# Ensembl/WiggleTools

Hardware: AMD Instinct MI355X
Metric: genomic bp/s (whole node) for 'mean' over N BigWig tracks (higher is better)
Workload: dtype f64

## Files before the change

include/wiggletools_amd.h:

```cpp
#ifndef WIGGLETOOLS_AMD_H_
#define WIGGLETOOLS_AMD_H_

#include <stdint.h>
#include <stdio.h>

#ifdef __cplusplus
extern "C" {
#endif


typedef char wt_bool;

typedef struct wiggleIterator_st WiggleIterator;
typedef struct multiplexer_st Multiplexer;
typedef struct multiset_st Multiset;

struct wiggleIterator_st {
    char *chrom;
    int start;
    int finish;
    double value;
    void *valuePtr;
    wt_bool done;
    int strand;
// ... 147 lines not shown
void wtamd_warmup_async(void);
const char *wtamd_last_error(void);
const char *wtamd_version(void);

#define WTAMD_MAX_COORD (2147483647 - 65536)

int wtamd_trackset_create_host(const wtamd_tracks *tracks, wtamd_trackset **out);
int wtamd_trackset_create_device(const wtamd_tracks *tracks, wtamd_trackset **out);
void wtamd_trackset_destroy(wtamd_trackset *);

int wtamd_trackset_validate(wtamd_trackset *ts, int64_t *n_bad, int64_t *first_bad);

int64_t wtamd_trackset_max_runs(const wtamd_trackset *ts);

int wtamd_trackset_index(wtamd_trackset *ts, int op, void *stream);

int wtamd_reduce(wtamd_trackset *ts, const wtamd_reduce_desc *desc, wtamd_runs *runs,
                 int64_t *n_runs, void *stream);

int wtamd_reduce_host(wtamd_trackset *ts, const wtamd_reduce_desc *desc, wtamd_runs *runs,
                      int64_t *n_runs);

int wtamd_multiplex_host(wtamd_trackset *ts, uint32_t flags, wtamd_runs *runs,
                         double *values, uint8_t *inplay, int64_t *n_runs);

int wtamd_runs_auc(const wtamd_runs *runs, int64_t n_runs, double *auc, void *stream);
int wtamd_runs_mean(const wtamd_runs *runs, int64_t n_runs, double *mean, void *stream);

int wtamd_pearson(wtamd_trackset *ts, double *result);
int wtamd_pearson_moments(wtamd_trackset *ts, double *moments6);
// ... 304 lines not shown
```

wiggletools_amd/_lib.py:

```python
import ctypes as C
import os

_HERE = os.path.dirname(os.path.abspath(__file__))
LIB_PATH = os.environ.get("WTAMD_LIB") or os.path.join(_HERE, "csrc", "libwiggletools_amd.so")


class Tracks(C.Structure):
    _fields_ = [("n_chrom", C.c_int32), ("n_tracks", C.c_int32), ("seg_off", C.c_void_p),
                ("start", C.c_void_p), ("finish", C.c_void_p), ("value", C.c_void_p),
                ("value_is_f64", C.c_int32), ("defaults", C.c_void_p),
                ("range_lo", C.c_void_p), ("range_hi", C.c_void_p)]


class ReduceDesc(C.Structure):
    _fields_ = [("op", C.c_int32), ("flags", C.c_uint32), ("n_set0", C.c_int32), ("reserved", C.c_int32)]


class Runs(C.Structure):
    _fields_ = [("capacity", C.c_int64), ("start", C.c_void_p), ("finish", C.c_void_p),
                ("value", C.c_void_p), ("chrom_run_off", C.c_void_p)]


class Stats(C.Structure):
    _fields_ = [("n_runs", C.c_int64), ("covered_bp", C.c_int64), ("n_intervals", C.c_int64),
# ... 15 lines not shown
    try:
        if os.environ.get("WTAMD_NO_TORCH"):
            raise ImportError
        import torch
    except ImportError:
        pass
    L = C.CDLL(LIB_PATH)
    L.wtamd_last_error.restype = C.c_char_p
    L.wtamd_version.restype = C.c_char_p
    L.wtamd_device_count.restype = C.c_int
    L.wtamd_set_device.argtypes = [C.c_int]
    L.wtamd_trackset_create_host.argtypes = [C.POINTER(Tracks), C.POINTER(C.c_void_p)]
    L.wtamd_trackset_create_device.argtypes = [C.POINTER(Tracks), C.POINTER(C.c_void_p)]
    L.wtamd_trackset_destroy.argtypes = [C.c_void_p]
    L.wtamd_trackset_destroy.restype = None
    L.wtamd_trackset_max_runs.argtypes = [C.c_void_p]
    L.wtamd_trackset_max_runs.restype = C.c_int64
    L.wtamd_trackset_index.argtypes = [C.c_void_p, C.c_int, C.c_void_p]
    L.wtamd_reduce.argtypes = [C.c_void_p, C.POINTER(ReduceDesc), C.POINTER(Runs), C.POINTER(C.c_int64), C.c_void_p]
    L.wtamd_reduce_host.argtypes = [C.c_void_p, C.POINTER(ReduceDesc), C.POINTER(Runs), C.POINTER(C.c_int64)]
    L.wtamd_multiplex_host.argtypes = [C.c_void_p, C.c_uint32, C.POINTER(Runs), C.c_void_p, C.c_void_p,
                                       C.POINTER(C.c_int64)]
    L.wtamd_runs_auc.argtypes = [C.POINTER(Runs), C.c_int64, C.POINTER(C.c_double), C.c_void_p]
    L.wtamd_runs_map.argtypes = [C.c_int, C.c_double, C.c_int64, C.c_void_p, C.c_void_p, C.c_void_p, C.c_void_p, C.c_int,
                                 C.c_void_p, C.c_void_p, C.c_void_p, C.c_void_p, C.c_void_p]
    L.wtamd_runs_coverage.argtypes = [C.c_int64, C.c_void_p, C.c_void_p, C.c_void_p, C.c_int64, C.c_void_p, C.c_void_p, C.c_void_p,
                                      C.c_void_p, C.POINTER(C.c_int64), C.c_void_p]
    L.wtamd_runs_union.argtypes = [C.c_int64, C.c_void_p, C.c_void_p, C.c_void_p, C.c_void_p, C.c_int, C.c_int64, C.c_void_p, C.c_void_p,
                                   C.c_void_p, C.c_void_p, C.POINTER(C.c_int64), C.c_void_p]
    L.wtamd_runs_region.argtypes = [C.c_int, C.c_int64, C.c_void_p, C.c_void_p, C.c_void_p, C.c_void_p, C.c_int, C.c_void_p, C.c_void_p,
# ... 70 lines not shown
```

wiggletools_amd/csrc/wt_engine.hip:

```cpp
#include <hip/hip_runtime.h>

#include <cstdio>
#include <thread>
#include <atomic>
#include <cstring>
#include <map>
#include <mutex>
#include <string>
#include <vector>

#include "wt_host.h"
#include "wt_trackset.h"
#include "wt_core.h"
#include "wt_plan.h"
#include "wt_kernels.h"
#include "wt_devscope.h"
#include "wt_pool.h"

#ifndef WT_INDEX_UNROLL
#define WT_INDEX_UNROLL 2
#endif
#define WT_INDEX_CHUNK (256 * 4 * WT_INDEX_UNROLL)
__global__ void __launch_bounds__(256) wt_index_kernel(const WtParams P, long long total, long long span) {
    const long long dev_total = P.seg_off[(long long) P.n_chrom * P.n_tracks];
    if (total > dev_total) total = dev_total;
    const long long begin0 = (long long) blockIdx.x * span;
    long long end0 = begin0 + span;
    if (end0 > total) end0 = total;
    if (begin0 >= end0) return;
    WtIndexCursor cur;
    wt_index_cursor_set(P, cur, wt_index_find_segment(P, begin0));
    struct __attribute__((packed, aligned(4))) V4 { int32_t x[4]; };
    V4 f[WT_INDEX_UNROLL], nf[WT_INDEX_UNROLL];
    int32_t pf[WT_INDEX_UNROLL], npf[WT_INDEX_UNROLL];
    const long long n_full = (end0 - begin0) / WT_INDEX_CHUNK;
    auto fetch = [&](long long base, V4 (&v)[WT_INDEX_UNROLL], int32_t (&p)[WT_INDEX_UNROLL]) {
#pragma unroll
        for (int u = 0; u < WT_INDEX_UNROLL; u++) {
// ... 29 lines not shown
            const long long g = begin + 4ll * (threadIdx.x + 256 * u);
            int32_t prev = (g < end0 && g > 0) ? P.finish[g - 1] : 0;
#pragma unroll
            for (int q = 0; q < 4; q++) {
                if (g + q < end0) {
                    const int32_t fq = P.finish[g + q];
                    wt_index_apply(P, cur, g + q, fq, prev);
                    prev = fq;
                }
            }
        }
    }
}

#define WT_ISEARCH_ROWS 64
#define WT_ISEARCH_TRACKS 16

__device__ __forceinline__ int wt_index_row_chrom(const WtParams &P, long long row) {
    int lo = 0;
    for (int hi = P.n_chrom; hi - lo > 1;) {
        const int mid = (lo + hi) >> 1;
        if (P.c_first_win[mid] + mid <= row) lo = mid; else hi = mid;
    }
    return lo;
}

struct WtIndexRow { int ch; long long b, s0, n; };
__device__ __forceinline__ WtIndexRow wt_index_row(const WtParams &P, long long row, int i) {
    WtIndexRow r;
    r.ch = P.n_chrom == 1 ? 0 : wt_index_row_chrom(P, row);
    const long long m = row - (P.c_first_win[r.ch] + r.ch);
    const long long seg = (long long) r.ch * P.n_tracks + i;
    r.s0 = P.seg_off[seg];
    r.n = P.seg_off[seg + 1] - r.s0;
    r.b = (long long) P.cbase[r.ch] + (m << P.logW);
    return r;
}

__global__ void __launch_bounds__(256) wt_index_coarse_kernel(const WtParams P, long long n_strips, uint32_t *coarse) {
    const long long t = (long long) blockIdx.x * 256 + threadIdx.x;
    const int N = P.n_tracks;
    if (t >= n_strips * N) return;
    const long long strip = t / N;
    const int i = (int) (t - strip * N);
    const WtIndexRow r = wt_index_row(P, strip * WT_ISEARCH_ROWS, i);
    const int32_t *fin = P.finish + r.s0;
    long long g = r.n >> 1;
    float density = 0.0f;
    if (r.n > 1) {
        const long long f0 = fin[0], f1 = fin[r.n - 1];
        if (f1 > f0) {
            density = (float) (r.n - 1) / (float) (f1 - f0);
            const float guess = fminf(fmaxf((float) (r.b - f0) * density, 0.0f), (float) (r.n - 1));
            g = (long long) guess;
            if (g > r.n - 1) g = r.n - 1;
        }
    }
    coarse[t] = (uint32_t) wt_interp_lower_bound(WtFinArray{fin}, 0, r.n, g, r.b, density);
}

__global__ void __launch_bounds__(WT_ISEARCH_ROWS * WT_ISEARCH_TRACKS) wt_index_search_kernel(const WtParams P, long long n_rows, long long n_strips,
                                                                                              const uint32_t *coarse) {
    __shared__ uint32_t out[WT_ISEARCH_ROWS][WT_ISEARCH_TRACKS + 1];
    const int tid = threadIdx.x, lane = tid & 63;
    const int wave = __builtin_amdgcn_readfirstlane(tid >> 6);
    const int N = P.n_tracks;
    const long long strip = blockIdx.x;
    const long long r0 = strip * WT_ISEARCH_ROWS;
    const int i = (int) blockIdx.y * WT_ISEARCH_TRACKS + wave;
    if (i < N) {
        long long row = r0 + lane;
        if (row > n_rows - 1) row = n_rows - 1;
        const WtIndexRow r = wt_index_row(P, row, i);
        const int32_t *fin = P.finish + r.s0;
        const bool have_next = strip + 1 < n_strips;
        const long long cA = (long long) coarse[strip * N + i];
        const long long cB = have_next ? (long long) coarse[(strip + 1) * N + i] : 0;
        bool real_a = true, real_b = have_next;
// ... 14 lines not shown
    const long long row = r0 + orow;
    const int track = (int) blockIdx.y * WT_ISEARCH_TRACKS + ocol;
    if (row < n_rows && track < N) P.widx[(size_t) row * N + track] = out[orow][ocol];
}

__global__ void __launch_bounds__(256) wt_index_compare_kernel(const uint32_t *a, const uint32_t *b, long long n, unsigned long long *diff) {
    const long long t = (long long) blockIdx.x * 256 + threadIdx.x;
    if (t < n && a[t] != b[t]) atomicAdd(diff, 1ull);
}

__global__ void __launch_bounds__(256) wt_extents_kernel(const int64_t *seg_off, const int32_t *start,
                                                          const int32_t *finish, long long n_seg,
                                                          int32_t *first_start, int32_t *last_finish) {
    const long long s = (long long) blockIdx.x * blockDim.x + threadIdx.x;
    if (s >= n_seg) return;
    const long long lo = seg_off[s], hi = seg_off[s + 1];
    first_start[s] = hi > lo ? start[lo] : 0;
    last_finish[s] = hi > lo ? finish[hi - 1] : 0;
}

__global__ void __launch_bounds__(256) wt_win_chrom_kernel(const int64_t *c_first_win, int n_chrom, long long n_windows, int32_t *win_chrom) {
    const long long k = (long long) blockIdx.x * 256 + threadIdx.x;
    if (k >= n_windows) return;
    int lo = 0;
    for (int hi = n_chrom; hi - lo > 1;) {
        const int mid = (lo + hi) >> 1;
        if (c_first_win[mid] <= k) lo = mid; else hi = mid;
    }
    win_chrom[k] = lo;
}

__global__ void __launch_bounds__(256) wt_clear_kernel(unsigned long long *counters, int n_counters, int64_t *chrom_run_off, int n_cro,
                                                        unsigned long long *status, long long n_status) {
    const long long t = (long long) blockIdx.x * 256 + threadIdx.x, stride = (long long) gridDim.x * 256;
    for (long long q = t; q < n_status; q += stride) status[q] = 0ull;
    for (long long q = t; q < n_counters; q += stride) counters[q] = 0ull;
    for (long long q = t; q < n_cro; q += stride) chrom_run_off[q] = 0;
}

__global__ void __launch_bounds__(256) wt_validate_kernel(const int32_t *start, const int32_t *finish, const int64_t *seg_off,
                                                           long long n_seg, long long total, unsigned long long *out) {
    const long long g = (long long) blockIdx.x * blockDim.x + threadIdx.x;
    if (g >= total) return;
    bool bad = finish[g] <= start[g];
    if (!bad && g > 0 && start[g] < finish[g - 1]) {
        long long lo = 0, hi = n_seg;
        while (hi - lo > 1) {
            const long long mid = (lo + hi) >> 1;
            if (seg_off[mid] <= g) lo = mid; else hi = mid;
        }
        bad = seg_off[lo] != g;
// ... 137 lines not shown
    WT_HIP(hipEventCreate(&ts->ev_r0));
    WT_HIP(hipEventCreate(&ts->ev_r1));
    return WTAMD_OK;
}

extern "C++" int wt_check_extents(wtamd_trackset *ts) {
    for (size_t q = 0; q < ts->last_finish.size(); q++)
        if (ts->seg_off[q + 1] > ts->seg_off[q] && ts->last_finish[q] > WTAMD_MAX_COORD) {
            const int64_t bad = ts->last_finish[q];
            return wt_fail(WTAMD_ERR_ARG, "run finish " + std::to_string(bad) + " above the supported maximum " +
                           std::to_string((long long) WTAMD_MAX_COORD) + " (2^31 - 65537)");
        }
    return WTAMD_OK;
}

static int wt_refresh_extents_device(wtamd_trackset *ts, hipStream_t s) {
    const int64_t n_seg = (int64_t) ts->n_chrom * ts->n_tracks;
    ts->first_start.assign(n_seg, 0);
    ts->last_finish.assign(n_seg, 0);
    if (n_seg > 0 && ts->n_intervals > 0) {
        const size_t bytes = sizeof(int32_t) * 2 * (size_t) n_seg;
        if (!ts->d_extents) WT_HIP(wt_dev_alloc(&ts->d_extents, bytes));
        if (!ts->h_extents) WT_HIP(wt_host_alloc((void **) &ts->h_extents, bytes));
        hipLaunchKernelGGL(wt_extents_kernel, dim3((unsigned) ((n_seg + 255) / 256)), dim3(256), 0, s,
                           ts->d_seg_off, ts->d_start, ts->d_finish, (long long) n_seg, ts->d_extents, ts->d_extents + n_seg);
        WT_HIP(hipGetLastError());
        WT_HIP(hipMemcpyAsync(ts->h_extents, ts->d_extents, bytes, hipMemcpyDeviceToHost, s));
        WT_HIP(hipStreamSynchronize(s));
        ts->first_start.assign(ts->h_extents, ts->h_extents + n_seg);
        ts->last_finish.assign(ts->h_extents + n_seg, ts->h_extents + 2 * n_seg);
    }
    return WTAMD_OK;
}

static int wt_create_host_impl(const wtamd_tracks *t, wtamd_trackset *ts) {
    int rc = wt_trackset_common(t, ts);
    if (rc != WTAMD_OK) return rc;
    ts->owns = true;
// ... 26 lines not shown
    const int rc = wt_create_host_impl(t, ts);
    if (rc != WTAMD_OK) { wtamd_trackset_destroy(ts); return rc; }
    *out = ts;
    return WTAMD_OK;
}

static int wt_create_device_impl(const wtamd_tracks *t, wtamd_trackset *ts) {
    int rc = wt_trackset_common(t, ts);
    if (rc != WTAMD_OK) return rc;
    ts->owns = false;
    ts->d_start = const_cast<int32_t *>(t->start);
    ts->d_finish = const_cast<int32_t *>(t->finish);
    ts->d_value = const_cast<void *>(t->value);
    rc = wt_refresh_extents_device(ts, nullptr);
    if (rc != WTAMD_OK) return rc;
    return wt_check_extents(ts);
}

int wtamd_trackset_create_device(const wtamd_tracks *t, wtamd_trackset **out) {
    if (!out) return wt_fail(WTAMD_ERR_ARG, "out == NULL");
    wtamd_trackset *ts = new wtamd_trackset();
    const int rc = wt_create_device_impl(t, ts);
    if (rc != WTAMD_OK) { wtamd_trackset_destroy(ts); return rc; }
    *out = ts;
    return WTAMD_OK;
}

void wtamd_trackset_destroy(wtamd_trackset *ts) {
    if (!ts) return;
    (void) wt_pool_quiesce();
    if (ts->owns) { (void) hipFree(ts->d_start); (void) hipFree(ts->d_finish); (void) hipFree(ts->d_value); }
    (void) wt_dev_free(ts->d_seg_off); (void) wt_dev_free(ts->d_defaults); (void) wt_dev_free(ts->d_counters); (void) wt_dev_free(ts->d_chrom_run_off);
    (void) wt_dev_free(ts->d_extents);
    (void) hipFree(ts->d_gscratch); (void) hipFree(ts->d_mwu_table);
    for (double *q : ts->mwu_retired) (void) hipFree(q);
    if (ts->h_counters) wt_host_free(ts->h_counters);
    if (ts->h_debug) wt_host_free(ts->h_debug);
    if (ts->h_extents) wt_host_free(ts->h_extents);
    for (auto &kv : ts->windows) wt_free_windows(kv.second);
    if (ts->ev_i0) (void) hipEventDestroy(ts->ev_i0);
    if (ts->ev_i1) (void) hipEventDestroy(ts->ev_i1);
    if (ts->ev_r0) (void) hipEventDestroy(ts->ev_r0);
    if (ts->ev_r1) (void) hipEventDestroy(ts->ev_r1);
    delete ts;
}

static int64_t wt_span(const wtamd_trackset *ts) {
    int64_t span = 0;
    for (int c = 0; c < ts->n_chrom; c++) {
        int64_t lo = INT64_MAX, hi = INT64_MIN;
        for (int i = 0; i < ts->n_tracks; i++) {
            const int64_t s = (int64_t) c * ts->n_tracks + i;
            if (ts->seg_off[s + 1] > ts->seg_off[s]) {
                lo = std::min<int64_t>(lo, ts->first_start[s]);
                hi = std::max<int64_t>(hi, ts->last_finish[s]);
            }
        }
        if (lo <= hi) span += hi - lo;
    }
    return span;
}

int64_t wtamd_trackset_max_runs(const wtamd_trackset *ts) {
    if (!ts) return 0;
    return std::min<int64_t>(2 * ts->n_intervals, wt_span(ts));
}

static int wt_get_windows(wtamd_trackset *ts, int W, WtWindows **out, hipStream_t s = nullptr) {
    WtWindows &w = ts->windows[W];
    *out = &w;
    if (w.tab_valid) return WTAMD_OK;
    wt_make_windows(ts->n_chrom, ts->n_tracks, ts->seg_off.data(), ts->first_start.data(), ts->last_finish.data(), W, w.tab,
                    ts->range_lo.empty() ? nullptr : ts->range_lo.data(),
                    ts->range_hi.empty() ? nullptr : ts->range_hi.data(), false);
    w.indexed = false;
    const int64_t nc = ts->n_chrom > 0 ? ts->n_chrom : 1;
    const int64_t nwin = w.tab.n_windows > 0 ? w.tab.n_windows : 1;
    const int64_t nwidx = (w.tab.n_rows > 0 ? w.tab.n_rows : 1) * (int64_t) ts->n_tracks;
    auto up8 = [](int64_t x) { return (x + 7) & ~(int64_t) 7; };
// ... 28 lines not shown
            w.h_tab = nullptr; w.h_tab_bytes = 0;
            WT_HIP(wt_host_alloc((void **) &w.h_tab, (size_t) head));
            w.h_tab_bytes = head;
        }
        const int64_t o_cfirst = (char *) w.d_cfirst - w.d_tabs;
        const int64_t used = o_cfirst + (int64_t) sizeof(int64_t) * (ts->n_chrom + 1);
        memset(w.h_tab, 0, (size_t) used);
        memcpy(w.h_tab + ((char *) w.d_cbase - w.d_tabs), w.tab.cbase.data(), sizeof(int32_t) * ts->n_chrom);
        memcpy(w.h_tab + ((char *) w.d_cnwin - w.d_tabs), w.tab.c_nwin.data(), sizeof(int32_t) * ts->n_chrom);
        memcpy(w.h_tab + ((char *) w.d_chi - w.d_tabs), w.tab.c_hi.data(), sizeof(int32_t) * ts->n_chrom);
        memcpy(w.h_tab + o_cfirst, w.tab.c_first_win.data(), sizeof(int64_t) * (ts->n_chrom + 1));
        WT_HIP(hipMemcpyAsync(w.d_tabs, w.h_tab, (size_t) used, hipMemcpyHostToDevice, s));
        WT_HIP(hipEventRecord(w.ev_tab, s));
        w.tab_in_flight = true;
        if (w.tab.n_windows > 0) {
            if (ts->n_chrom == 1) {
                WT_HIP(hipMemsetAsync(w.d_win_chrom, 0, sizeof(int32_t) * (size_t) w.tab.n_windows, s));
            } else {
                hipLaunchKernelGGL(wt_win_chrom_kernel, dim3((unsigned) ((w.tab.n_windows + 255) / 256)), dim3(256), 0, s,
                                   (const int64_t *) w.d_cfirst, ts->n_chrom, (long long) w.tab.n_windows, w.d_win_chrom);
                WT_HIP(hipGetLastError());
            }
        }
    }
    w.tab_valid = true;
    return WTAMD_OK;
}

static void wt_fill_params(const wtamd_trackset *ts, const WtWindows *w, const WtPlan &plan, WtParams &P) {
    memset(&P, 0, sizeof(P));
    P.start = ts->d_start; P.finish = ts->d_finish; P.value = ts->d_value;
    P.seg_off = ts->d_seg_off; P.defaults = ts->d_defaults;
    P.n_chrom = ts->n_chrom; P.n_tracks = ts->n_tracks; P.n_total = ts->n_intervals;
    P.cbase = w->d_cbase; P.c_nwin = w->d_cnwin; P.c_hi = w->d_chi; P.c_first_win = w->d_cfirst;
    P.n_windows = w->tab.n_windows; P.win_chrom = w->d_win_chrom; P.widx = w->d_widx;
    P.status = w->d_status; P.counters = ts->d_counters; P.debug = ts->h_debug;
    wt_plan_to_params(plan, P);
}

static int wt_build_index(wtamd_trackset *ts, WtWindows *w, const WtPlan &plan, hipStream_t s) {
    WtParams P;
    wt_fill_params(ts, w, plan, P);
    WT_HIP(hipEventRecord(ts->ev_i0, s));
    static const int mode = [] {
        const char *e = getenv("WTAMD_INDEX"), *c = getenv("WTAMD_INDEX_CHECK");
        if (c && atoi(c) > 0) return 2;
        return (e && !strcmp(e, "scan")) ? 1 : 0;
    }();
    const size_t n_widx = (size_t) w->tab.n_rows * ts->n_tracks;
    auto scan = [&](uint32_t *dst) -> int {
        WtParams Q = P;
        Q.widx = dst;
        WT_HIP(hipMemsetAsync(dst, 0, sizeof(uint32_t) * n_widx, s));
        if (ts->n_intervals > 0) {
            const long long total = ts->n_intervals;
            long long blocks = (total + WT_INDEX_CHUNK - 1) / WT_INDEX_CHUNK;
            const long long cap = (long long) ts->num_cu * 8;
            if (blocks > cap) blocks = cap;
            long long span = (total + blocks - 1) / blocks;
            span = (span + WT_INDEX_CHUNK - 1) / WT_INDEX_CHUNK * WT_INDEX_CHUNK;
            blocks = (total + span - 1) / span;
            hipLaunchKernelGGL(wt_index_kernel, dim3((unsigned) blocks), dim3(256), 0, s, Q, total, span);
            WT_HIP(hipGetLastError());
        }
        return WTAMD_OK;
    };
    auto search = [&](uint32_t *dst) -> int {
        WtParams Q = P;
        Q.widx = dst;
        const long long n_rows = w->tab.n_rows;
        if (n_rows > 0 && ts->n_tracks > 0) {
            const long long n_strips = (n_rows + WT_ISEARCH_ROWS - 1) / WT_ISEARCH_ROWS;
            if (w->cap_cidx < n_strips * ts->n_tracks) return wt_fail(WTAMD_ERR_INTERNAL, "coarse window index not allocated");
            hipLaunchKernelGGL(wt_index_coarse_kernel, dim3((unsigned) ((n_strips * ts->n_tracks + 255) / 256)), dim3(256), 0, s, Q, n_strips, w->d_cidx);
            WT_HIP(hipGetLastError());
            const dim3 grid((unsigned) n_strips, (unsigned) ((ts->n_tracks + WT_ISEARCH_TRACKS - 1) / WT_ISEARCH_TRACKS));
            hipLaunchKernelGGL(wt_index_search_kernel, grid, dim3(WT_ISEARCH_ROWS * WT_ISEARCH_TRACKS), 0, s, Q, n_rows, n_strips, (const uint32_t *) w->d_cidx);
            WT_HIP(hipGetLastError());
        }
        return WTAMD_OK;
    };
    if (mode == 1) {
        if (int rc = scan(w->d_widx)) return rc;
    } else {
        if (int rc = search(w->d_widx)) return rc;
    }
    if (mode == 2 && n_widx > 0) {
        uint32_t *other = nullptr;
        unsigned long long *d_diff = nullptr, h_diff = 0;
        WT_HIP(hipMalloc(&other, sizeof(uint32_t) * n_widx));
        WT_HIP(hipMalloc(&d_diff, sizeof(unsigned long long)));
        WT_HIP(hipMemsetAsync(d_diff, 0, sizeof(unsigned long long), s));
// ... 53 lines not shown

extern "C++" int wt_trackset_rebind(wtamd_trackset *ts, int64_t n, const int64_t *seg_off, int32_t range_lo, int32_t range_hi, bool value_f64,
                                    int32_t *d_start, int32_t *d_finish, void *d_value, bool delta_failed) {
    ts->n_intervals = n;
    ts->seg_off.assign(seg_off, seg_off + (int64_t) ts->n_chrom * ts->n_tracks + 1);
    ts->range_lo[0] = range_lo;
    ts->range_hi[0] = range_hi;
    ts->value_f64 = value_f64;
    ts->scratch_f32 = !ts->value_f64 && wt_defaults_fit_f32(ts->defaults.data(), ts->n_tracks);
    ts->d_start = d_start; ts->d_finish = d_finish; ts->d_value = d_value;
    wt_trackset_forget(ts, delta_failed);
    for (auto &kv : ts->windows) kv.second.tab_valid = false;
    return wt_check_extents(ts);
}

int wtamd_trackset_index(wtamd_trackset *ts, int op, void *stream) {
    if (!ts) return wt_fail(WTAMD_ERR_ARG, "ts == NULL");
    wt_trackset_forget(ts, false);
    ts->mwu_few_ties = -1;
    if (!ts->owns && !ts->pipe_mode) {
        int rce = wt_refresh_extents_device(ts, (hipStream_t) stream);
        if (rce != WTAMD_OK) return rce;
        rce = wt_check_extents(ts);
        if (rce != WTAMD_OK) return rce;
        for (auto &kv : ts->windows) kv.second.tab_valid = false;
    }
    WtPlan plan;
    std::string err;
    if (wt_wants_delta(ts, op)) wt_make_delta_plan_for(plan, ts->n_tracks, op);
    else if (!wt_pick_plan(ts, op, ts->n_tracks / 2, plan, err, (hipStream_t) stream)) return wt_fail(WTAMD_ERR_ARG, err);
    WtWindows *w = nullptr;
    int rc = wt_get_windows(ts, plan.W, &w, (hipStream_t) stream);
    if (rc != WTAMD_OK) return rc;
    return wt_build_index(ts, w, plan, (hipStream_t) stream);
}

extern "C++" int wt_check_desc(const wtamd_trackset *ts, const wtamd_reduce_desc *d) {
    if (!ts || !d) return wt_fail(WTAMD_ERR_ARG, "NULL argument");
    if (d->op < 0 || d->op >= WTAMD_OP_COUNT_) return wt_fail(WTAMD_ERR_ARG, "unknown op");
    if (d->op == WTAMD_OP_TTEST) {
        if (d->n_set0 < 3 || ts->n_tracks - d->n_set0 < 3)
            return wt_fail(WTAMD_ERR_ARG, "The t-test function only works for two sets with enough elements to compute variance");
    } else if (d->op == WTAMD_OP_MWU) {
// ... 35 lines not shown
    Q.ratio = delta_W / plan.W;
    if (!wt_patch_launch(L, Q, op, plan.ppt, plan.n_chunks > 1, n_bad, !w->indexed))
        return wt_fail(WTAMD_ERR_INTERNAL, "no general plan compatible with the difference-array windows");
    if (L.err != hipSuccess) return wt_fail(WTAMD_ERR_HIP, std::string("patch kernel launch: ") + hipGetErrorString(L.err));
    WT_HIP(hipEventRecord(ts->ev_r1, s));
    ts->stats.patched_windows = (int32_t) n_bad;
    return WTAMD_OK;
}

static int wt_reduce_impl(wtamd_trackset *ts, int op, uint32_t flags, int n_set0, wtamd_runs *runs,
                          double *d_tile, uint8_t *d_inplay, int64_t *n_runs, hipStream_t s) {
    if (!runs || !runs->start || !runs->finish || !runs->value)
        return wt_fail(WTAMD_ERR_ARG, "wtamd_reduce: output arrays missing");
    WtPlan plan;
    std::string err;
    if (!d_tile && wt_wants_delta(ts, op)) {
        wt_make_delta_plan_for(plan, ts->n_tracks, op);
        const int dc = wt_delta_class(op);
        int64_t n_probe = 0;
        const bool probe = !ts->delta_verified_[dc];
        const int rc = wt_reduce_plan(ts, plan, op, flags, n_set0, runs, d_tile, d_inplay,
                                      (probe && !n_runs) ? &n_probe : n_runs, s);
        if (!probe) {
            if (ts->delta_n_bad_[dc] > 0 && (rc == WTAMD_OK || rc == WTAMD_ERR_CAPACITY)) {
                const int rp = wt_launch_patch(ts, plan.W, op, flags, n_set0, runs, ts->delta_n_bad_[dc], s);
                if (rp != WTAMD_OK) return rp;
                if (n_runs) WT_HIP(hipStreamSynchronize(s));
            }
            return rc;
        }
        if (rc != WTAMD_OK && rc != WTAMD_ERR_CAPACITY) return rc;
        const long long n_bad = (long long) ts->h_counters[WT_CTR_DELTA_BAD];
        if (n_bad == 0) { ts->delta_verified_[dc] = true; ts->delta_n_bad_[dc] = 0; return rc; }
        if (wt_few_enough_to_patch(n_bad, ts->stats.n_windows) && !getenv("WTAMD_NO_PATCH")) {
            const int rp = wt_launch_patch(ts, plan.W, op, flags, n_set0, runs, n_bad, s);
            if (rp == WTAMD_OK) {
                WT_HIP(hipStreamSynchronize(s));
// ... 65 lines not shown
            bool quiet = false;
            WT_HIP(wt_grow(&w->d_bad_list, &c1, nwin, &quiet));
            WT_HIP(wt_grow(&w->d_bad_goff, &c2, nwin * WT_BAD_SUB, &quiet));
            w->cap_bad = c1 < c2 / WT_BAD_SUB ? c1 : c2 / WT_BAD_SUB;
        }
        L.P.bad_list = w->d_bad_list;
        L.P.bad_goff = w->d_bad_goff;
        wt_delta_defaults_params(ts->defaults.data(), ts->n_tracks, L.P);
    }

    const bool launches = w->tab.n_windows > 0 && ts->n_intervals > 0;
    {
        const long long n_status = launches ? (long long) w->tab.n_windows : 0;
        const long long most = std::max<long long>(std::max<long long>(n_status, WT_CTR_N), ts->n_chrom + 1);
        const unsigned blocks = (unsigned) std::min<long long>((most + 255) / 256, 1024);
        hipLaunchKernelGGL(wt_clear_kernel, dim3(blocks), dim3(256), 0, s, ts->d_counters, (int) WT_CTR_N, L.P.chrom_run_off, ts->n_chrom + 1,
                           w->d_status, n_status);
        WT_HIP(hipGetLastError());
    }
    if (launches) {
        if (plan.delta) {
            static const int force_u = getenv("WTAMD_DELTA_U") ? atoi(getenv("WTAMD_DELTA_U")) : 0;
            const double tiles_per_wave = (double) ts->n_intervals / (double) w->tab.n_windows / 256.0 / (double) std::max(1, L.T / 64);
            L.small_tiles = force_u == 2 || (force_u != 4 && tiles_per_wave < 8.0);
        }
        WT_HIP(hipEventRecord(ts->ev_r0, s));
        if (plan.delta) {
            wt_delta_launch(L, op);
        } else if (plan.walk_S) {
            L.err = wt_walk_launch(L.P, plan.regcol, L.T, L.lds, L.num_cu, L.gscratch, L.gscratch_bytes, L.stream, &L.grid);
        } else if (!wt_reduce_launch(L, op, ts->value_f64, ts->scratch_f32, plan.ppt, plan.n_chunks > 1 || plan.scratch_slab > 0, plan.regcol)) {
            return wt_fail(WTAMD_ERR_ARG, "op not dispatchable");
// ... 196 lines not shown
    WT_HIP(scope.alloc(&d, sizeof h));
    WT_HIP(hipMemcpy(d, h, sizeof h, hipMemcpyHostToDevice));
    const long long total = ts->n_intervals;
    hipLaunchKernelGGL(wt_validate_kernel, dim3((unsigned) ((total + 255) / 256)), dim3(256), 0, nullptr, ts->d_start,
                       ts->d_finish, ts->d_seg_off, (long long) ts->n_chrom * ts->n_tracks, total, d);
    const hipError_t e = hipMemcpy(h, d, sizeof h, hipMemcpyDeviceToHost);
    if (e != hipSuccess) return wt_fail(WTAMD_ERR_HIP, "wtamd_trackset_validate: kernel / copy failed");
    *n_bad = (int64_t) h[0];
    if (first_bad && h[0]) *first_bad = (int64_t) h[1];
    return WTAMD_OK;
}

int wtamd_get_stats(const wtamd_trackset *ts_c, wtamd_stats *out) {
    if (!ts_c || !out) return wt_fail(WTAMD_ERR_ARG, "NULL argument");
    wtamd_trackset *ts = const_cast<wtamd_trackset *>(ts_c);
    if (ts->have_index_time && hipEventSynchronize(ts->ev_i1) == hipSuccess)
        (void) hipEventElapsedTime(&ts->stats.index_ms, ts->ev_i0, ts->ev_i1);
    if (ts->have_reduce_time && hipEventSynchronize(ts->ev_r1) == hipSuccess)
        (void) hipEventElapsedTime(&ts->stats.reduce_ms, ts->ev_r0, ts->ev_r1);
    *out = ts->stats;
    return WTAMD_OK;
}

}
```

wiggletools_amd/csrc/wt_trackset.h:

```cpp
#ifndef WT_TRACKSET_H_
#define WT_TRACKSET_H_

#include <map>
#include <vector>

#include "wt_host.h"
#include "wt_plan.h"

struct WtWindows {
    WtPlan plan_geom;
    WtWindowTables tab;
    int32_t *d_cbase = nullptr, *d_cnwin = nullptr, *d_chi = nullptr, *d_win_chrom = nullptr;
    int64_t *d_cfirst = nullptr;
    uint32_t *d_widx = nullptr;
    uint32_t *d_cidx = nullptr;
    unsigned long long *d_status = nullptr;
    int32_t *d_bad_list = nullptr;
    long long *d_bad_goff = nullptr;
    bool indexed = false;
    int64_t cap_chrom = 0, cap_win = 0, cap_widx = 0, cap_bad = 0, cap_cidx = 0;
    bool tab_valid = false;
    char *h_tab = nullptr;
    int64_t h_tab_bytes = 0;
    hipEvent_t ev_tab = nullptr;
// ... 8 lines not shown
    bool owns = false;
    int64_t n_intervals = 0;
    std::vector<int64_t> seg_off;
    std::vector<double> defaults;
    std::vector<int32_t> first_start, last_finish;
    std::vector<int32_t> range_lo, range_hi;
    int32_t *d_start = nullptr, *d_finish = nullptr;
    void *d_value = nullptr;
    int64_t *d_seg_off = nullptr;
    double *d_defaults = nullptr;
    unsigned long long *d_counters = nullptr;
    unsigned long long *h_counters = nullptr;
    unsigned long long *h_debug = nullptr;
    int64_t *d_chrom_run_off = nullptr;
    int32_t *d_extents = nullptr, *h_extents = nullptr;
    char *d_gscratch = nullptr;
    size_t gscratch_bytes = 0;
    double *d_mwu_table = nullptr;
    int mwu_n1 = -1, mwu_n2 = -1, mwu_kmax = 0;
    int mwu_few_ties = -1;
    std::vector<double *> mwu_retired;
    std::map<int, WtWindows> windows;
    hipEvent_t ev_i0 = nullptr, ev_i1 = nullptr, ev_r0 = nullptr, ev_r1 = nullptr;
    bool have_index_time = false, have_reduce_time = false;
    wtamd_stats stats{};
    int device = 0;
    int num_cu = 256;
    bool scratch_f32 = false;
    bool delta_failed_[3] = {false, false, false};
    bool delta_verified_[3] = {false, false, false};
    long long delta_n_bad_[3] = {0, 0, 0};
    bool pipe_mode = false;
};

void wt_warmup_join();
int wt_trackset_common(const wtamd_tracks *t, wtamd_trackset *ts);
int wt_check_extents(wtamd_trackset *ts);
int wt_check_desc(const wtamd_trackset *ts, const wtamd_reduce_desc *d);

int wt_trackset_rebind(wtamd_trackset *ts, int64_t n, const int64_t *seg_off, int32_t range_lo, int32_t range_hi, bool value_f64,
                       int32_t *d_start, int32_t *d_finish, void *d_value, bool delta_failed);

int wt_reduce_enqueue(wtamd_trackset *ts, const wtamd_reduce_desc &desc, wtamd_runs *runs, double *d_tile, uint8_t *d_inplay,
                      hipStream_t s, bool *used_delta, int *delta_W);

int wt_launch_patch(wtamd_trackset *ts, int delta_W, int op, uint32_t flags, int n_set0, wtamd_runs *runs, long long n_bad,
                    hipStream_t s);

#endif
```

wiggletools_amd/engine.py:

```python
import ctypes as C

import numpy as np

from . import _lib
from .runlists import RunLists

OPS = {"sum": 0, "product": 1, "mult": 1, "mean": 2, "var": 3, "stddev": 4, "entropy": 5, "cv": 6, "CV": 6,
       "min": 7, "max": 8, "median": 9, "ttest": 10, "mwu": 11, "wilcoxon": 11}
STRICT_SET0, STRICT_SET1 = 1, 2
STATS = {"var": 0, "stddev": 1, "cv": 2, "CV": 2, "max": 3, "min": 4, "span": 5}


def opcode(op):
    if isinstance(op, str):
        if op not in OPS:
            raise ValueError("unknown reducer %r" % op)
        return OPS[op]
    return int(op)


def reducer_default(op, defaults):
    d = np.ascontiguousarray(defaults, np.float64)
    return _lib.lib().wtamd_reducer_default(opcode(op), len(d), d.ctypes.data)

# ... 344 lines not shown
            _lib.lib().wtamd_trackset_destroy(self._h)
            self._h = None

    def __del__(self):
        try:
            self.close()
        except Exception:
            pass

    def max_runs(self):
        return int(_lib.lib().wtamd_trackset_max_runs(self._h))

    def index(self, op="mean", stream=None):
        _lib.check(_lib.lib().wtamd_trackset_index(self._h, opcode(op), stream))

    def stats(self):
        s = _lib.Stats()
        _lib.check(_lib.lib().wtamd_get_stats(self._h, C.byref(s)))
        return {k: getattr(s, k) for k, _ in _lib.Stats._fields_}

    def validate(self):
        n, first = C.c_int64(), C.c_int64()
        _lib.check(_lib.lib().wtamd_trackset_validate(self._h, C.byref(n), C.byref(first)))
        return n.value, first.value

    def pearson(self):
        out = C.c_double()
        _lib.check(_lib.lib().wtamd_pearson(self._h, C.byref(out)))
        return out.value

# ... 125 lines not shown
```

Measured before the change: 49.64 billion.

## Verify segment extents speculatively on device instead of blocking host refresh in index

Before, indexing a borrowed track set read the segment extents back to the host synchronously before it could build the window index. Now a single-block kernel recomputes the extents on the device, compares them with the held copy and writes a changed flag to mapped host memory. Index, clear and reduce kernels are queued speculatively and skip work or poison the ticket counter when the flag is set. The host settles the verdict lazily and reruns the index and reduce if the extents changed. This removes a host-device round trip from the index path, at the cost of much more complex state handling and a possible second reduce.

```diff
diff --git a/include/wiggletools_amd.h b/include/wiggletools_amd.h
--- a/include/wiggletools_amd.h
+++ b/include/wiggletools_amd.h
@@ -185,6 +185,7 @@
 int64_t wtamd_trackset_max_runs(const wtamd_trackset *ts);
 
 int wtamd_trackset_index(wtamd_trackset *ts, int op, void *stream);
+int wtamd_trackset_unsettled(const wtamd_trackset *ts);
 
 int wtamd_reduce(wtamd_trackset *ts, const wtamd_reduce_desc *desc, wtamd_runs *runs,
                  int64_t *n_runs, void *stream);
diff --git a/wiggletools_amd/_lib.py b/wiggletools_amd/_lib.py
--- a/wiggletools_amd/_lib.py
+++ b/wiggletools_amd/_lib.py
@@ -53,6 +53,7 @@
     L.wtamd_trackset_create_device.argtypes = [C.POINTER(Tracks), C.POINTER(C.c_void_p)]
     L.wtamd_trackset_destroy.argtypes = [C.c_void_p]
     L.wtamd_trackset_destroy.restype = None
+    L.wtamd_trackset_unsettled.argtypes = [C.c_void_p]
     L.wtamd_trackset_max_runs.argtypes = [C.c_void_p]
     L.wtamd_trackset_max_runs.restype = C.c_int64
     L.wtamd_trackset_index.argtypes = [C.c_void_p, C.c_int, C.c_void_p]
diff --git a/wiggletools_amd/csrc/wt_engine.hip b/wiggletools_amd/csrc/wt_engine.hip
--- a/wiggletools_amd/csrc/wt_engine.hip
+++ b/wiggletools_amd/csrc/wt_engine.hip
@@ -16,12 +16,14 @@
 #include "wt_kernels.h"
 #include "wt_devscope.h"
 #include "wt_pool.h"
+#include "wt_extents.h"
 
 #ifndef WT_INDEX_UNROLL
 #define WT_INDEX_UNROLL 2
 #endif
 #define WT_INDEX_CHUNK (256 * 4 * WT_INDEX_UNROLL)
-__global__ void __launch_bounds__(256) wt_index_kernel(const WtParams P, long long total, long long span) {
+__global__ void __launch_bounds__(256) wt_index_kernel(const WtParams P, long long total, long long span, const int32_t *changed) {
+    if (changed && *changed) return;
     const long long dev_total = P.seg_off[(long long) P.n_chrom * P.n_tracks];
     if (total > dev_total) total = dev_total;
     const long long begin0 = (long long) blockIdx.x * span;
@@ -81,6 +83,7 @@
 }
 
 #define WT_ISEARCH_ROWS 64
+#define WT_TICKET_POISON (1ull << 62)
 #define WT_ISEARCH_TRACKS 16
 
 __device__ __forceinline__ int wt_index_row_chrom(const WtParams &P, long long row) {
@@ -104,7 +107,8 @@
     return r;
 }
 
-__global__ void __launch_bounds__(256) wt_index_coarse_kernel(const WtParams P, long long n_strips, uint32_t *coarse) {
+__global__ void __launch_bounds__(256) wt_index_coarse_kernel(const WtParams P, long long n_strips, uint32_t *coarse, const int32_t *changed) {
+    if (changed && *changed) return;
     const long long t = (long long) blockIdx.x * 256 + threadIdx.x;
     const int N = P.n_tracks;
     if (t >= n_strips * N) return;
@@ -127,8 +131,9 @@
 }
 
 __global__ void __launch_bounds__(WT_ISEARCH_ROWS * WT_ISEARCH_TRACKS) wt_index_search_kernel(const WtParams P, long long n_rows, long long n_strips,
-                                                                                              const uint32_t *coarse) {
+                                                                                              const uint32_t *coarse, const int32_t *changed) {
     __shared__ uint32_t out[WT_ISEARCH_ROWS][WT_ISEARCH_TRACKS + 1];
+    if (changed && *changed) return;
     const int tid = threadIdx.x, lane = tid & 63;
     const int wave = __builtin_amdgcn_readfirstlane(tid >> 6);
     const int N = P.n_tracks;
@@ -173,9 +178,25 @@
                                                           int32_t *first_start, int32_t *last_finish) {
     const long long s = (long long) blockIdx.x * blockDim.x + threadIdx.x;
     if (s >= n_seg) return;
-    const long long lo = seg_off[s], hi = seg_off[s + 1];
-    first_start[s] = hi > lo ? start[lo] : 0;
-    last_finish[s] = hi > lo ? finish[hi - 1] : 0;
+    wt_segment_extents(seg_off, start, finish, s, &first_start[s], &last_finish[s]);
+}
+
+__global__ void __launch_bounds__(1024) wt_extents_verify_kernel(const int64_t *seg_off, const int32_t *start, const int32_t *finish,
+                                                                  long long n_seg, const int32_t *held, int32_t *fresh, int32_t *pinned) {
+    int differ = 0;
+    for (long long s = threadIdx.x; s < n_seg; s += blockDim.x) {
+        int32_t fs, lf;
+        wt_segment_extents(seg_off, start, finish, s, &fs, &lf);
+        fresh[s] = fs; fresh[n_seg + s] = lf;
+        pinned[s] = fs; pinned[n_seg + s] = lf;
+        differ |= (fs != held[s]) | (lf != held[n_seg + s]);
+    }
+    const int any = __syncthreads_or(differ);
+    if (threadIdx.x == 0) {
+        fresh[2 * n_seg] = any ? 1 : 0;
+        pinned[2 * n_seg] = any ? 1 : 0;
+    }
+    __threadfence_system();
 }
 
 __global__ void __launch_bounds__(256) wt_win_chrom_kernel(const int64_t *c_first_win, int n_chrom, long long n_windows, int32_t *win_chrom) {
@@ -190,10 +211,11 @@
 }
 
 __global__ void __launch_bounds__(256) wt_clear_kernel(unsigned long long *counters, int n_counters, int64_t *chrom_run_off, int n_cro,
-                                                        unsigned long long *status, long long n_status) {
+                                                        unsigned long long *status, long long n_status, const int32_t *changed) {
     const long long t = (long long) blockIdx.x * 256 + threadIdx.x, stride = (long long) gridDim.x * 256;
+    const unsigned long long ticket0 = (changed && *changed) ? WT_TICKET_POISON : 0ull;
     for (long long q = t; q < n_status; q += stride) status[q] = 0ull;
-    for (long long q = t; q < n_counters; q += stride) counters[q] = 0ull;
+    for (long long q = t; q < n_counters; q += stride) counters[q] = q == WT_CTR_TICKET ? ticket0 : 0ull;
     for (long long q = t; q < n_cro; q += stride) chrom_run_off[q] = 0;
 }
 
@@ -361,14 +383,23 @@
     return WTAMD_OK;
 }
 
+static int wt_extents_buffers(wtamd_trackset *ts) {
+    const size_t bytes = sizeof(int32_t) * wt_extents_words((int64_t) ts->n_chrom * ts->n_tracks);
+    if (!ts->d_extents) WT_HIP(wt_dev_alloc(&ts->d_extents, bytes));
+    if (!ts->d_extents2) WT_HIP(wt_dev_alloc(&ts->d_extents2, bytes));
+    if (!ts->h_extents) WT_HIP(wt_host_alloc((void **) &ts->h_extents, bytes));
+    if (!ts->ev_ext) WT_HIP(hipEventCreateWithFlags(&ts->ev_ext, hipEventDisableTiming));
+    return WTAMD_OK;
+}
+
 static int wt_refresh_extents_device(wtamd_trackset *ts, hipStream_t s) {
     const int64_t n_seg = (int64_t) ts->n_chrom * ts->n_tracks;
+    ts->ext_valid = false;
     ts->first_start.assign(n_seg, 0);
     ts->last_finish.assign(n_seg, 0);
     if (n_seg > 0 && ts->n_intervals > 0) {
         const size_t bytes = sizeof(int32_t) * 2 * (size_t) n_seg;
-        if (!ts->d_extents) WT_HIP(wt_dev_alloc(&ts->d_extents, bytes));
-        if (!ts->h_extents) WT_HIP(wt_host_alloc((void **) &ts->h_extents, bytes));
+        if (int rcb = wt_extents_buffers(ts)) return rcb;
         hipLaunchKernelGGL(wt_extents_kernel, dim3((unsigned) ((n_seg + 255) / 256)), dim3(256), 0, s,
                            ts->d_seg_off, ts->d_start, ts->d_finish, (long long) n_seg, ts->d_extents, ts->d_extents + n_seg);
         WT_HIP(hipGetLastError());
@@ -425,7 +456,9 @@
     ts->d_value = const_cast<void *>(t->value);
     rc = wt_refresh_extents_device(ts, nullptr);
     if (rc != WTAMD_OK) return rc;
-    return wt_check_extents(ts);
+    rc = wt_check_extents(ts);
+    ts->ext_valid = rc == WTAMD_OK;
+    return rc;
 }
 
 int wtamd_trackset_create_device(const wtamd_tracks *t, wtamd_trackset **out) {
@@ -442,7 +475,7 @@
     (void) wt_pool_quiesce();
     if (ts->owns) { (void) hipFree(ts->d_start); (void) hipFree(ts->d_finish); (void) hipFree(ts->d_value); }
     (void) wt_dev_free(ts->d_seg_off); (void) wt_dev_free(ts->d_defaults); (void) wt_dev_free(ts->d_counters); (void) wt_dev_free(ts->d_chrom_run_off);
-    (void) wt_dev_free(ts->d_extents);
+    (void) wt_dev_free(ts->d_extents); (void) wt_dev_free(ts->d_extents2);
     (void) hipFree(ts->d_gscratch); (void) hipFree(ts->d_mwu_table);
     for (double *q : ts->mwu_retired) (void) hipFree(q);
     if (ts->h_counters) wt_host_free(ts->h_counters);
@@ -453,6 +486,7 @@
     if (ts->ev_i1) (void) hipEventDestroy(ts->ev_i1);
     if (ts->ev_r0) (void) hipEventDestroy(ts->ev_r0);
     if (ts->ev_r1) (void) hipEventDestroy(ts->ev_r1);
+    if (ts->ev_ext) (void) hipEventDestroy(ts->ev_ext);
     delete ts;
 }
 
@@ -474,6 +508,7 @@
 
 int64_t wtamd_trackset_max_runs(const wtamd_trackset *ts) {
     if (!ts) return 0;
+    if (wt_settle_extents(const_cast<wtamd_trackset *>(ts)) != WTAMD_OK) return 0;
     return std::min<int64_t>(2 * ts->n_intervals, wt_span(ts));
 }
 
@@ -532,7 +567,7 @@
         WT_HIP(hipEventRecord(w.ev_tab, s));
         w.tab_in_flight = true;
         if (w.tab.n_windows > 0) {
-            if (ts->n_chrom == 1) {
+            if (ts->n_chrom == 1 && ts->pipe_mode) {
                 WT_HIP(hipMemsetAsync(w.d_win_chrom, 0, sizeof(int32_t) * (size_t) w.tab.n_windows, s));
             } else {
                 hipLaunchKernelGGL(wt_win_chrom_kernel, dim3((unsigned) ((w.tab.n_windows + 255) / 256)), dim3(256), 0, s,
@@ -556,15 +591,20 @@
     wt_plan_to_params(plan, P);
 }
 
-static int wt_build_index(wtamd_trackset *ts, WtWindows *w, const WtPlan &plan, hipStream_t s) {
-    WtParams P;
-    wt_fill_params(ts, w, plan, P);
-    WT_HIP(hipEventRecord(ts->ev_i0, s));
+static int wt_index_mode() {
     static const int mode = [] {
         const char *e = getenv("WTAMD_INDEX"), *c = getenv("WTAMD_INDEX_CHECK");
         if (c && atoi(c) > 0) return 2;
         return (e && !strcmp(e, "scan")) ? 1 : 0;
     }();
+    return mode;
+}
+
+static int wt_build_index(wtamd_trackset *ts, WtWindows *w, const WtPlan &plan, hipStream_t s, const int32_t *changed = nullptr) {
+    WtParams P;
+    wt_fill_params(ts, w, plan, P);
+    WT_HIP(hipEventRecord(ts->ev_i0, s));
+    const int mode = wt_index_mode();
     const size_t n_widx = (size_t) w->tab.n_rows * ts->n_tracks;
     auto scan = [&](uint32_t *dst) -> int {
         WtParams Q = P;
@@ -578,7 +618,7 @@
             long long span = (total + blocks - 1) / blocks;
             span = (span + WT_INDEX_CHUNK - 1) / WT_INDEX_CHUNK * WT_INDEX_CHUNK;
             blocks = (total + span - 1) / span;
-            hipLaunchKernelGGL(wt_index_kernel, dim3((unsigned) blocks), dim3(256), 0, s, Q, total, span);
+            hipLaunchKernelGGL(wt_index_kernel, dim3((unsigned) blocks), dim3(256), 0, s, Q, total, span, changed);
             WT_HIP(hipGetLastError());
         }
         return WTAMD_OK;
@@ -590,10 +630,10 @@
         if (n_rows > 0 && ts->n_tracks > 0) {
             const long long n_strips = (n_rows + WT_ISEARCH_ROWS - 1) / WT_ISEARCH_ROWS;
             if (w->cap_cidx < n_strips * ts->n_tracks) return wt_fail(WTAMD_ERR_INTERNAL, "coarse window index not allocated");
-            hipLaunchKernelGGL(wt_index_coarse_kernel, dim3((unsigned) ((n_strips * ts->n_tracks + 255) / 256)), dim3(256), 0, s, Q, n_strips, w->d_cidx);
+            hipLaunchKernelGGL(wt_index_coarse_kernel, dim3((unsigned) ((n_strips * ts->n_tracks + 255) / 256)), dim3(256), 0, s, Q, n_strips, w->d_cidx, changed);
             WT_HIP(hipGetLastError());
             const dim3 grid((unsigned) n_strips, (unsigned) ((ts->n_tracks + WT_ISEARCH_TRACKS - 1) / WT_ISEARCH_TRACKS));
-            hipLaunchKernelGGL(wt_index_search_kernel, grid, dim3(WT_ISEARCH_ROWS * WT_ISEARCH_TRACKS), 0, s, Q, n_rows, n_strips, (const uint32_t *) w->d_cidx);
+            hipLaunchKernelGGL(wt_index_search_kernel, grid, dim3(WT_ISEARCH_ROWS * WT_ISEARCH_TRACKS), 0, s, Q, n_rows, n_strips, (const uint32_t *) w->d_cidx, changed);
             WT_HIP(hipGetLastError());
         }
         return WTAMD_OK;
@@ -677,19 +717,78 @@
     return wt_check_extents(ts);
 }
 
+extern "C++" int wt_settle_extents(wtamd_trackset *ts, bool *changed) {
+    if (changed) *changed = false;
+    if (ts->ext_error) return wt_fail(ts->ext_error, ts->ext_error_msg);
+    if (!ts->ext_pending) return WTAMD_OK;
+    ts->ext_pending = false;
+    WT_HIP(hipEventSynchronize(ts->ev_ext));
+    const int64_t n_seg = (int64_t) ts->n_chrom * ts->n_tracks;
+    const bool differ = ts->h_extents[2 * n_seg] != 0;
+    if (differ == wt_extents_same(ts->first_start.data(), ts->last_finish.data(), ts->h_extents, n_seg)) {
+        ts->ext_valid = false;
+        return wt_fail(WTAMD_ERR_INTERNAL, "extents verdict of the device contradicts the extents it wrote");
+    }
+    if (!differ) return WTAMD_OK;
+    if (changed) *changed = true;
+    const hipStream_t s = ts->ext_stream;
+    wt_extents_adopt(ts->h_extents, n_seg, ts->first_start, ts->last_finish);
+    WT_HIP(hipMemcpyAsync(ts->d_extents, ts->d_extents2, sizeof(int32_t) * 2 * (size_t) n_seg, hipMemcpyDeviceToDevice, s));
+    for (auto &kv : ts->windows) { kv.second.tab_valid = false; kv.second.indexed = false; }
+    ts->ext_valid = false;
+    if (wt_check_extents(ts) != WTAMD_OK) {
+        ts->ext_error = WTAMD_ERR_ARG;
+        ts->ext_error_msg = g_last_error;
+        return ts->ext_error;
+    }
+    ts->ext_valid = true;
+    WtPlan plan;
+    wt_make_delta_plan_for(plan, ts->n_tracks, ts->ext_op);
+    WtWindows *w = nullptr;
+    const int rc = wt_get_windows(ts, plan.W, &w, s);
+    if (rc != WTAMD_OK) return rc;
+    return wt_build_index(ts, w, plan, s);
+}
+
+int wtamd_trackset_unsettled(const wtamd_trackset *ts) { return ts && ts->ext_pending ? 1 : 0; }
+
 int wtamd_trackset_index(wtamd_trackset *ts, int op, void *stream) {
     if (!ts) return wt_fail(WTAMD_ERR_ARG, "ts == NULL");
+    ts->ext_error = 0;
+    (void) wt_settle_extents(ts);
+    ts->ext_error = 0;
     wt_trackset_forget(ts, false);
     ts->mwu_few_ties = -1;
+    WtPlan plan;
+    std::string err;
     if (!ts->owns && !ts->pipe_mode) {
+        const bool sync_forced = getenv("WTAMD_INDEX_SYNC") && atoi(getenv("WTAMD_INDEX_SYNC")) > 0;
+        const bool mapped = sizeof(int32_t) * wt_extents_words((int64_t) ts->n_chrom * ts->n_tracks) < ((size_t) 1 << 20);
+        if (!sync_forced && mapped && ts->ext_valid && ts->d_extents2 && ts->n_intervals > 0 && wt_index_mode() != 2 && wt_wants_delta(ts, op)) {
+            const hipStream_t s = (hipStream_t) stream;
+            const long long n_seg = (long long) ts->n_chrom * ts->n_tracks;
+            hipLaunchKernelGGL(wt_extents_verify_kernel, dim3(1), dim3(1024), 0, s, ts->d_seg_off, ts->d_start, ts->d_finish, n_seg,
+                               (const int32_t *) ts->d_extents, ts->d_extents2, ts->h_extents);
+            WT_HIP(hipGetLastError());
+            WT_HIP(hipEventRecord(ts->ev_ext, s));
+            ts->ext_pending = true; ts->ext_op = op; ts->ext_stream = s;
+            wt_make_delta_plan_for(plan, ts->n_tracks, op);
+            WtWindows *w = nullptr;
+            const int rc = wt_get_windows(ts, plan.W, &w, s);
+            if (rc != WTAMD_OK) return rc;
+            return wt_build_index(ts, w, plan, s, ts->d_extents2 + 2 * n_seg);
+        }
         int rce = wt_refresh_extents_device(ts, (hipStream_t) stream);
         if (rce != WTAMD_OK) return rce;
+        for (auto &kv : ts->windows) kv.second.tab_valid = false;
         rce = wt_check_extents(ts);
-        if (rce != WTAMD_OK) return rce;
-        for (auto &kv : ts->windows) kv.second.tab_valid = false;
-    }
-    WtPlan plan;
-    std::string err;
+        if (rce != WTAMD_OK) {
+            ts->ext_error = rce;
+            ts->ext_error_msg = g_last_error;
+            return rce;
+        }
+        ts->ext_valid = true;
+    }
     if (wt_wants_delta(ts, op)) wt_make_delta_plan_for(plan, ts->n_tracks, op);
     else if (!wt_pick_plan(ts, op, ts->n_tracks / 2, plan, err, (hipStream_t) stream)) return wt_fail(WTAMD_ERR_ARG, err);
     WtWindows *w = nullptr;
@@ -755,13 +854,31 @@
         return wt_fail(WTAMD_ERR_ARG, "wtamd_reduce: output arrays missing");
     WtPlan plan;
     std::string err;
+    bool unsettled = false;
+    if (ts->ext_pending || ts->ext_error) {
+        if (ts->ext_pending && !d_tile && s == ts->ext_stream && wt_wants_delta(ts, op) && !ts->delta_verified_[wt_delta_class(op)]) {
+            wt_make_delta_plan_for(plan, ts->n_tracks, op);
+            const auto it = ts->windows.find(plan.W);
+            unsettled = it != ts->windows.end() && it->second.tab_valid && it->second.indexed;
+        }
+        if (!unsettled) {
+            const int rcs = wt_settle_extents(ts);
+            if (rcs != WTAMD_OK) return rcs;
+        }
+    }
     if (!d_tile && wt_wants_delta(ts, op)) {
         wt_make_delta_plan_for(plan, ts->n_tracks, op);
         const int dc = wt_delta_class(op);
         int64_t n_probe = 0;
         const bool probe = !ts->delta_verified_[dc];
-        const int rc = wt_reduce_plan(ts, plan, op, flags, n_set0, runs, d_tile, d_inplay,
-                                      (probe && !n_runs) ? &n_probe : n_runs, s);
+        int rc = wt_reduce_plan(ts, plan, op, flags, n_set0, runs, d_tile, d_inplay,
+                                (probe && !n_runs) ? &n_probe : n_runs, s);
+        if (unsettled) {
+            bool changed = false;
+            const int rcs = wt_settle_extents(ts, &changed);
+            if (rcs != WTAMD_OK) return rcs;
+            if (changed) rc = wt_reduce_plan(ts, plan, op, flags, n_set0, runs, d_tile, d_inplay, (probe && !n_runs) ? &n_probe : n_runs, s);
+        }
         if (!probe) {
             if (ts->delta_n_bad_[dc] > 0 && (rc == WTAMD_OK || rc == WTAMD_ERR_CAPACITY)) {
                 const int rp = wt_launch_patch(ts, plan.W, op, flags, n_set0, runs, ts->delta_n_bad_[dc], s);
@@ -857,8 +974,10 @@
         const long long n_status = launches ? (long long) w->tab.n_windows : 0;
         const long long most = std::max<long long>(std::max<long long>(n_status, WT_CTR_N), ts->n_chrom + 1);
         const unsigned blocks = (unsigned) std::min<long long>((most + 255) / 256, 1024);
+        const int32_t *changed = ts->ext_pending ? ts->d_extents2 + 2 * (size_t) ts->n_chrom * ts->n_tracks : nullptr;
+        if (changed && !plan.delta) return wt_fail(WTAMD_ERR_INTERNAL, "a launch that takes no tickets on a track set with unsettled extents");
         hipLaunchKernelGGL(wt_clear_kernel, dim3(blocks), dim3(256), 0, s, ts->d_counters, (int) WT_CTR_N, L.P.chrom_run_off, ts->n_chrom + 1,
-                           w->d_status, n_status);
+                           w->d_status, n_status, changed);
         WT_HIP(hipGetLastError());
     }
     if (launches) {
@@ -1085,6 +1204,7 @@
 int wtamd_get_stats(const wtamd_trackset *ts_c, wtamd_stats *out) {
     if (!ts_c || !out) return wt_fail(WTAMD_ERR_ARG, "NULL argument");
     wtamd_trackset *ts = const_cast<wtamd_trackset *>(ts_c);
+    if (const int rcs = wt_settle_extents(ts)) return rcs;
     if (ts->have_index_time && hipEventSynchronize(ts->ev_i1) == hipSuccess)
         (void) hipEventElapsedTime(&ts->stats.index_ms, ts->ev_i0, ts->ev_i1);
     if (ts->have_reduce_time && hipEventSynchronize(ts->ev_r1) == hipSuccess)
diff --git a/wiggletools_amd/csrc/wt_extents.h b/wiggletools_amd/csrc/wt_extents.h
--- /dev/null
+++ b/wiggletools_amd/csrc/wt_extents.h
@@ -0,0 +1,40 @@
+#ifndef WT_EXTENTS_H_
+#define WT_EXTENTS_H_
+
+#include <cstdint>
+#include <cstddef>
+#include <vector>
+
+#include "wt_plan.h"
+
+#if defined(__HIPCC__) && !defined(WT_EMU)
+#define WT_EXT_HD __host__ __device__ __forceinline__
+#else
+#define WT_EXT_HD inline
+#endif
+
+static inline size_t wt_extents_words(int64_t n_seg) { return 2 * (size_t) n_seg + 1; }
+
+WT_EXT_HD void wt_segment_extents(const int64_t *seg_off, const int32_t *start, const int32_t *finish, long long s, int32_t *fs, int32_t *lf) {
+    const long long lo = seg_off[s], hi = seg_off[s + 1];
+    *fs = hi > lo ? start[lo] : 0;
+    *lf = hi > lo ? finish[hi - 1] : 0;
+}
+
+static inline bool wt_extents_same(const int32_t *held_first, const int32_t *held_last, const int32_t *fresh, int64_t n_seg) {
+    for (int64_t s = 0; s < n_seg; s++)
+        if (held_first[s] != fresh[s] || held_last[s] != fresh[n_seg + s]) return false;
+    return true;
+}
+
+static inline void wt_extents_adopt(const int32_t *fresh, int64_t n_seg, std::vector<int32_t> &first_start, std::vector<int32_t> &last_finish) {
+    first_start.assign(fresh, fresh + n_seg);
+    last_finish.assign(fresh + n_seg, fresh + 2 * n_seg);
+}
+
+static inline bool wt_windows_same(const WtWindowTables &a, const WtWindowTables &b) {
+    return a.n_windows == b.n_windows && a.n_rows == b.n_rows && a.span_bp == b.span_bp && a.cbase == b.cbase && a.c_nwin == b.c_nwin &&
+           a.c_hi == b.c_hi && a.c_first_win == b.c_first_win && a.win_chrom == b.win_chrom && a.empty_chrom == b.empty_chrom;
+}
+
+#endif
diff --git a/wiggletools_amd/csrc/wt_trackset.h b/wiggletools_amd/csrc/wt_trackset.h
--- a/wiggletools_amd/csrc/wt_trackset.h
+++ b/wiggletools_amd/csrc/wt_trackset.h
@@ -46,6 +46,14 @@
     unsigned long long *h_debug = nullptr;
     int64_t *d_chrom_run_off = nullptr;
     int32_t *d_extents = nullptr, *h_extents = nullptr;
+    int32_t *d_extents2 = nullptr;
+    hipEvent_t ev_ext = nullptr;
+    bool ext_valid = false;
+    bool ext_pending = false;
+    int ext_op = 0;
+    hipStream_t ext_stream = nullptr;
+    int ext_error = 0;
+    std::string ext_error_msg;
     char *d_gscratch = nullptr;
     size_t gscratch_bytes = 0;
     double *d_mwu_table = nullptr;
@@ -69,6 +77,7 @@
 int wt_trackset_common(const wtamd_tracks *t, wtamd_trackset *ts);
 int wt_check_extents(wtamd_trackset *ts);
 int wt_check_desc(const wtamd_trackset *ts, const wtamd_reduce_desc *d);
+int wt_settle_extents(wtamd_trackset *ts, bool *changed = nullptr);
 
 int wt_trackset_rebind(wtamd_trackset *ts, int64_t n, const int64_t *seg_off, int32_t range_lo, int32_t range_hi, bool value_f64,
                        int32_t *d_start, int32_t *d_finish, void *d_value, bool delta_failed);
diff --git a/wiggletools_amd/engine.py b/wiggletools_amd/engine.py
--- a/wiggletools_amd/engine.py
+++ b/wiggletools_amd/engine.py
@@ -382,6 +382,9 @@
     def index(self, op="mean", stream=None):
         _lib.check(_lib.lib().wtamd_trackset_index(self._h, opcode(op), stream))
 
+    def unsettled(self):
+        return bool(_lib.lib().wtamd_trackset_unsettled(self._h))
+
     def stats(self):
         s = _lib.Stats()
         _lib.check(_lib.lib().wtamd_get_stats(self._h, C.byref(s)))
```

Result: no change. 49.85 billion, median of 6 (+0.4%).
